# jbrea/BayesianOptimization.jl

Measured on AMD Instinct MI355X. Metric: acquisition-candidates/sec (N=3000,d=8), higher is better.
Workload: dtype f64

## Files before the change

### bayesianoptimization.jl_amd/csrc/bohip.hip

```cpp
#include "../../include/bohip.h"
#include "../../include/bohip_paths.h"
#include "../../include/bohip_fit.h"
#include "../../include/bohip_qei.h"
#include "../../include/bohip_acq.h"
#include "../../include/bohip_kg.h"
#include "../../include/bohip_ens.h"
#include "kernels_linalg.hip"
#include "kernels_chol.hip"
#include "kernels_exec.hip"
#include "kernels_score.hip"
#include "kernels_batch.hip"
#include "kernels_sample.hip"
#include "kernels_qei.hip"
#include "kernels_kg.hip"
#include "kernels_path.hip"
#include "kernels_ascent.hip"
#include "kernels_fit.hip"
#include "kernels_ens.hip"
#include "kernels_small.hip"
#include "direct_l.h"

#include <algorithm>
#include <atomic>
#include <chrono>
// ... 292 lines not shown
    HIPCHK(hipMalloc(&g->dr, (g->ld + 256) * 8));
    HIPCHK(hipMalloc(&g->dt, (g->ld + 256) * 8));
    HIPCHK(hipMalloc(&g->dApp, (size_t)APP_ROWS * g->ld * 8));
    {
        const size_t Tm = (size_t)(g->ld / TILE) + 1;
        HIPCHK(hipMalloc(&g->dchol_flags, chol_flag_words((int)std::min<size_t>(Tm, CHOL_DF_TCAP)) * sizeof(unsigned)));
        HIPCHK(hipMalloc(&g->dchol_idl, Tm * CH_PANELS * 256 * 8));
    }
    HIPCHK(hipMemsetAsync(g->dL, 0, mat, g->stream));
    HIPCHK(hipMemsetAsync(g->dW, 0, mat, g->stream));
    HIPCHK(hipMemsetAsync(g->dWT, 0, mat, g->stream));
    HIPCHK(hipMemsetAsync(g->dS, 0, mat, g->stream));
    if (g->n > 0) {
        HIPCHK(hipMemcpyAsync(g->dX, g->hX.data(), (size_t)g->n * g->d * 8, hipMemcpyHostToDevice, g->stream));
        HIPCHK(hipMemcpyAsync(g->dy, g->hy.data(), (size_t)g->n * 8, hipMemcpyHostToDevice, g->stream));
    }
    g->stale = true;
    return 0;
}

static int g_bulk_pieces = 4;
static int g_sample_mfma_min = 200;
static int g_path_mfma_min = 24;
static int g_split = 1;
static int g_asc_wg_nmax = 256;
static const double g_asc_first_step = 0.1;
static int g_asc_fold = 1;
static int g_asc_lockstep = 0;
static int g_small_m = 0;
static int g_small_r = -1;
static int g_inv_hi_h = 16;
static int g_chol_df = 1;
static bool g_chol_df_strict = false;
static bool g_chol_df_dump = false;
static int g_chol_df_tmax = 96;
static std::atomic<int> g_chol_df_skip{0}, g_chol_df_backoff{0};
static unsigned long long g_chol_spin_ticks = CH_SPIN_TICKS_DEFAULT;
static int g_chol_exec_patience_us = 1000;
static int g_chol_exec_fill_inv = 1;
static int g_chol_exec_inv_pairs = 0;
static std::atomic<int> g_chol_inv_grp_min{28};
static std::atomic<int> g_chol_inv_g{8};
static int g_chol_nsf = 3;
static int g_chol_exec_urgent = -1;
static int g_chol_exec_second = 1;
static int g_small_zero_copy = 1;
static int g_chol_exec_nbu = 2;
static int g_chol_exec_fast = -1;
static int g_chol_exec_pairs = -1;
static int g_chol_exec_wgs = -1;
static int g_append_alpha_inc = 1;
static int64_t g_chunk_rows_forced = 0;
static int g_prune_m = -1;
static int g_pa_order = 1;
static int launch_gemm_nt(bohip_gp* g, const GemmNTParams& p, int batch = 1, hipStream_t st = nullptr, bool hi = false) {
    if (p.mt <= 0 || p.nt64 <= 0 || p.kc <= 0 || batch <= 0) return 0;
    if (hi) hipLaunchKernelGGL(k_gemm_nt_hi, dim3(p.mt * p.nt64, batch), dim3(GEMM_THREADS_8), glds3_lds_bytes<4>(), st ? st : g->stream, p);
    else hipLaunchKernelGGL(k_gemm_nt, dim3(p.mt * p.nt64, batch), dim3(GEMM_THREADS_8), glds3_lds_bytes<4>(), st ? st : g->stream, p);
    HIPCHK(hipGetLastError());
    return 0;
}

static int device_cus();
static void read_dev_knobs() {
#if BOHIP_DEV_KNOBS
    struct Knob { const char* name; int* v; int lo, hi; };
    static int chunk_rows = 0, dump = 0;
    const Knob knobs[] = {
        {"BOHIP_CHOL_DF_TMAX", &g_chol_df_tmax, 0, CHOL_DF_TCAP}, {"BOHIP_INV_HI_H", &g_inv_hi_h, 0, 1 << 20},
        {"BOHIP_CHOL_EXEC_PAIRS", &g_chol_exec_pairs, -1, 64},
        {"BOHIP_CHOL_EXEC_URGENT", &g_chol_exec_urgent, 1, 1 << 20}, {"BOHIP_CHOL_NSF", &g_chol_nsf, 1, CH_NSF_MAX},
        {"BOHIP_CHOL_EXEC_PATIENCE_US", &g_chol_exec_patience_us, 0, 1 << 30}, {"BOHIP_CHOL_EXEC_FILL_INV", &g_chol_exec_fill_inv, 0, 1},
        {"BOHIP_CHOL_EXEC_INV_PAIRS", &g_chol_exec_inv_pairs, 0, 1}, {"BOHIP_CHOL_EXEC_WGS", &g_chol_exec_wgs, 1, 1 << 20},
        {"BOHIP_CHOL_EXEC_FAST", &g_chol_exec_fast, -1, 1 << 20},
        {"BOHIP_CHOL_EXEC_SECOND", &g_chol_exec_second, 0, 1}, {"BOHIP_SMALL_ZERO_COPY", &g_small_zero_copy, 0, 1}, {"BOHIP_CHOL_EXEC_NBU", &g_chol_exec_nbu, 0, 16}, {"BOHIP_CHUNK_ROWS", &chunk_rows, 0, 1 << 30},
        {"BOHIP_PRUNE_M", &g_prune_m, -1, 1 << 16}, {"BOHIP_PA_ORDER", &g_pa_order, 0, 1},
        {"BOHIP_APPEND_ALPHA_INC", &g_append_alpha_inc, 0, 1}, {"BOHIP_BULK_PIECES", &g_bulk_pieces, 0, 8}, {"BOHIP_SPLIT", &g_split, 0, 1},
        {"BOHIP_SMALL_R", &g_small_r, 0, SMALL_MAX}, {"BOHIP_SMALL_M", &g_small_m, 0, 1 << 20}, {"BOHIP_CHOL_DF_DUMP", &dump, 0, 1},
    };
    for (const Knob& k : knobs)
        if (const char* e = getenv(k.name)) *k.v = std::min(k.hi, std::max(k.lo, atoi(e)));
    g_chunk_rows_forced = chunk_rows;
    g_chol_df_dump = dump != 0;
#endif
}

static int one_time_kernel_setup() {
    static bool done_dev[64] = {false};
    int dev = 0;
    HIPCHK(hipGetDevice(&dev));
    bool& done = done_dev[dev & 63];
    if (done) return 0;
    HIPCHK(hipFuncSetAttribute((const void*)k_potf2_inv, hipFuncAttributeMaxDynamicSharedMemorySize, POTF2_LDS_BYTES));
    HIPCHK(hipFuncSetAttribute((const void*)k_gemm_nt, hipFuncAttributeMaxDynamicSharedMemorySize, glds3_lds_bytes<4>()));
    HIPCHK(hipFuncSetAttribute((const void*)k_trigemm_sq, hipFuncAttributeMaxDynamicSharedMemorySize, glds3_lds_bytes<4>()));
    HIPCHK(hipFuncSetAttribute((const void*)k_trigemm_sq_pa, hipFuncAttributeMaxDynamicSharedMemorySize, glds3_lds_bytes<4>()));
    HIPCHK(hipFuncSetAttribute((const void*)k_trigemm_rows, hipFuncAttributeMaxDynamicSharedMemorySize, RS_LDS_BYTES));
    HIPCHK(hipFuncSetAttribute((const void*)k_batch_cond<true>, hipFuncAttributeMaxDynamicSharedMemorySize, BATCH_LDS_MAX));
    HIPCHK(hipFuncSetAttribute((const void*)k_batch_cond<false>, hipFuncAttributeMaxDynamicSharedMemorySize, BATCH_LDS_MAX));
    HIPCHK(hipFuncSetAttribute((const void*)k_chol_chain, hipFuncAttributeMaxDynamicSharedMemorySize, CH_LDS_BYTES));
    HIPCHK(hipFuncSetAttribute((const void*)k_gemm_nt_hi, hipFuncAttributeMaxDynamicSharedMemorySize, glds3_lds_bytes<4>()));
    HIPCHK(hipFuncSetAttribute((const void*)k_chol_exec, hipFuncAttributeMaxDynamicSharedMemorySize, glds3_lds_bytes<4>()));
    HIPCHK(hipFuncSetAttribute((const void*)k_trimv_stream<TRIMV_D>, hipFuncAttributeMaxDynamicSharedMemorySize, trimv_lds_bytes(TRIMV_D)));
    HIPCHK(hipFuncSetAttribute((const void*)k_path_mfma<true>, hipFuncAttributeMaxDynamicSharedMemorySize, (int)path_mfma_lds_bytes(DMAX)));
    HIPCHK(hipFuncSetAttribute((const void*)k_path_mfma<false>, hipFuncAttributeMaxDynamicSharedMemorySize, (int)path_mfma_lds_bytes(DMAX)));
    HIPCHK(hipFuncSetAttribute((const void*)k_kg<true>, hipFuncAttributeMaxDynamicSharedMemorySize, (int)kg_lds_bytes(KG_RMAX)));
    HIPCHK(hipFuncSetAttribute((const void*)k_kg<false>, hipFuncAttributeMaxDynamicSharedMemorySize, (int)kg_lds_bytes(KG_RMAX)));
    if (const char* e = getenv("BOHIP_CHOL_DATAFLOW")) g_chol_df = atoi(e);
    if (const char* e = getenv("BOHIP_CHOL_SPIN_US")) g_chol_spin_ticks = 100ull * (unsigned long long)std::max(1, atoi(e));
    if (const char* e = getenv("BOHIP_CHOL_INV_G")) g_chol_inv_g = std::min(64, std::max(0, atoi(e)));
    if (const char* e = getenv("BOHIP_CHOL_INV_GRP_MIN")) g_chol_inv_grp_min = std::max(0, atoi(e));
    if (const char* e = getenv("BOHIP_ASC_WG_NMAX")) g_asc_wg_nmax = std::max(0, atoi(e));
    if (const char* e = getenv("BOHIP_ASC_LOCKSTEP")) { g_asc_lockstep = atoi(e) == 1; g_asc_fold = atoi(e) != 2; }
    if (const char* e = getenv("BOHIP_SAMPLE_MFMA_MIN")) g_sample_mfma_min = std::max(1, atoi(e));
    g_chol_df_strict = getenv("BOHIP_CHOL_DF_STRICT") != nullptr;
    read_dev_knobs();
    done = true;
    return 0;
}

static int launch_rows_trimv(bohip_gp* g, const double* W, int64_t N0, const double* rows, int P, double* out, int upper);
static int compute_alpha(bohip_gp* g) {
    const int64_t N = g->n;
    g->alpha_inc_run = 0;
    hipLaunchKernelGGL(k_sub_mean, dim3((N + 255) / 256), dim3(256), 0, g->stream, g->dy, g->beta, N, g->dr);
    HIPCHK(hipGetLastError());
    CHK(launch_rows_trimv(g, g->dW, N, g->dr, 1, g->dt, 0));
    CHK(launch_rows_trimv(g, g->dWT, N, g->dt, 1, g->dalpha, 1));
    HIPCHK(hipMemcpyAsync(g->dW + N * g->ld, g->dalpha, (size_t)N * 8, hipMemcpyDeviceToDevice, g->stream));
    return 0;
}

static int check_info(bohip_gp* g) {
    int info = 0;
    if (g->hpin) {
        int* pw = reinterpret_cast<int*>(g->hpin + 3 * SMALL_R) + 1;
        HIPCHK(hipMemcpyAsync(pw, g->dinfo, sizeof(int), hipMemcpyDeviceToHost, g->stream));
        HIPCHK(hipStreamSynchronize(g->stream));
        info = *pw;
    } else {
        HIPCHK(hipMemcpyAsync(&info, g->dinfo, sizeof(int), hipMemcpyDeviceToHost, g->stream));
        HIPCHK(hipStreamSynchronize(g->stream));
    }
    if (info != 0) {
        g->pivot = info;
        g->stale = true;
        return fail(BOHIP_E_NOTPD, "kernel matrix not positive definite at pivot " + std::to_string(info));
    }
    g->pivot = 0;
// ... 1142 lines not shown
static int prune_tiles(int T) {
    if (g_prune_m >= 0) return g_prune_m < T ? g_prune_m : 0;
    int m = 2;
    while ((double)m * (m + 1) < 0.02 * T * (T + 1)) ++m;
    return m < T ? m : 0;
}
static std::vector<int> rows_halves(const std::vector<int>& pieces) {
    std::vector<int> out;
    for (int c : pieces) {
        const int rt = c & 0xffff, mode = c >> 16;
        if (mode == PIECE_UPPER_SOLO) out.push_back(rt | 1 << 17);
        else { out.push_back(rt | 1 << 16); out.push_back(rt); }
    }
    std::stable_sort(out.begin(), out.end(), [](int a, int b) {
        return 8 * (a & 0xffff) + ((a >> 16) & 1) * 4 > 8 * (b & 0xffff) + ((b >> 16) & 1) * 4;
    });
    return out;
}
static int rows_halves_from(const std::vector<int>& hv, int t0) {
    int n = 0;
    while (n < (int)hv.size() && (hv[n] & 0xffff) >= t0) ++n;
    return n;
}
static int launch_trigemm_rows(bohip_gp* g, const double* KsT, const int* halves, int NH, const int* list, const unsigned* cnt,
                               int cnt_max, double* q, int64_t ldq, double* mu, int groups = 0, const PruneFinish* pf = nullptr,
                               unsigned* arrive = nullptr) {
    if (NH <= 0 || cnt_max <= 0) return 0;
    RowsParams rp{};
    rp.W = g->dW; rp.ldw = g->ld; rp.KsT = KsT; rp.ldk = g->ld; rp.list = list; rp.cnt = cnt; rp.cnt_max = cnt_max;
    rp.halves = halves; rp.NH = NH; rp.G = groups > 0 ? groups : (cnt_max + RS_COLS - 1) / RS_COLS;
    rp.alpha_row = g->n; rp.q = q; rp.ldq = ldq; rp.mu = mu;
    if (pf) { rp.finish = 1; rp.arrive = arrive; rp.pf = *pf; }
    hipLaunchKernelGGL(k_trigemm_rows, dim3((unsigned)(8 * ((NH + 7) / 8) * rp.G)), dim3(RS_THREADS), RS_LDS_BYTES, g->stream, rp);
    HIPCHK(hipGetLastError());
    return 0;
}
static int launch_trigemm_on(bohip_gp* g, const double* KsT, const int* pieces, int NP, int CT, double* q, int64_t ldq, double* mu_raw,
                             FuseParams fz) {
    const int n_local = (CT + 7) / 8;
    if (NP <= 0 || CT <= 0) return 0;
    if (g->timing && g->dclk) fz.clk = g->dclk;
    hipLaunchKernelGGL(k_trigemm_sq, dim3(8 * n_local * NP), dim3(GEMM_THREADS_8), glds3_lds_bytes<4>(), g->stream, g->dW, g->ld, KsT,
                       g->ld, pieces, NP, CT, g->n, q, ldq, mu_raw, (int64_t)0, nullptr, g->ld, fz);
    HIPCHK(hipGetLastError());
    return 0;
}
static std::vector<int> phase_a_jobs(const std::vector<int>& pieces, int m) {
    std::vector<int> out;
    for (int c : pieces)
        if ((c & 0xffff) < m) { out.push_back((c & 0xffff) | 1 << 16); out.push_back(c & 0xffff); }
    std::stable_sort(out.begin(), out.end(), [](int a, int b) {
        return 8 * (a & 0xffff) + (a >> 16) * 4 > 8 * (b & 0xffff) + (b >> 16) * 4;
    });
    if (g_pa_order == 1) std::rotate(out.begin(), out.begin() + out.size() / 3, out.begin() + 2 * (out.size() / 3));
    return out;
}
static int launch_phase_a(bohip_gp* g, const double* KsT, const int* jobs, int NJOBS, int CT, double* q, int64_t ldq) {
    const int n_local = (CT + 7) / 8;
    if (NJOBS <= 0 || CT <= 0) return 0;
    hipLaunchKernelGGL(k_trigemm_sq_pa, dim3(8 * n_local * NJOBS), dim3(GEMM_THREADS_8), glds3_lds_bytes<4>(), g->stream, g->dW, g->ld,
                       KsT, g->ld, jobs, CT, q, ldq, g->timing && g->dclk ? g->dclk : nullptr);
    HIPCHK(hipGetLastError());
    return 0;
}
static int pruned_pass(bohip_gp* g, const double* dXs, int64_t R, int m, const AcqParams& ap, Best* d_best, int64_t best_off,
                       double* ub_host = nullptr, bool long_form = false) {
    CHK(one_time_kernel_setup());
    if (!g->hprune_stat) {
        HIPCHK(hipHostMalloc((void**)&g->hprune_stat, 64, hipHostMallocDefault));
        g->hprune_stat[0] = 0u;
    }
    const int64_t N = g->n, Npad = round_up(N + 1, TILE), Rpad = round_up(R, TILE) + TILE, ld = g->ld;
    const int T = (int)(Npad / TILE);
    const int64_t P = Npad / 64;
    CHK(ensure_pieces(g, T, N));
    std::vector<int> pa, pb;
    for (int c : g->hpieces) ((c & 0xffff) < m ? pa : pb).push_back(c);
    if (m >= T) return fail(BOHIP_E_STATE, "pruned pass: the prefix holds the alpha row");
    for (int c : pa)
        if (c >> 16 != PIECE_WHOLE) return fail(BOHIP_E_STATE, "pruned pass: a half piece in the prefix");
    const std::vector<int> ph = phase_a_jobs(g->hpieces, m);
    auto al = [](size_t b) { return (b + 255) / 256 * 256; };
    const size_t o_ks = 0, o_q2 = o_ks + al((size_t)Rpad * ld * 8), o_mu2 = o_q2 + al((size_t)2 * T * Rpad * 8),
                 o_ub = o_mu2 + al((size_t)Rpad * 8), o_l1 = o_ub + al((size_t)Rpad * 8), o_l2 = o_l1 + al((size_t)PRUNE_K1 * 4),
                 o_mark = o_l2 + al((size_t)Rpad * 4), o_cnt = o_mark + al((size_t)Rpad * 4), o_rec = o_cnt + 256,
                 o_parts = o_rec + 256, o_pc = o_parts + al((size_t)2 * P * Rpad * 8), total = o_pc + al((5 * g->hpieces.size() + 8) * 4);
    bool fresh = false;
    if (g->pr_bytes < total) {
        fresh = true;
        if (g->dpr) { HIPCHK(hipStreamSynchronize(g->stream)); HIPCHK(hipFree(g->dpr)); g->dpr = nullptr; g->pr_bytes = 0; }
        HIPCHK(hipMalloc(&g->dpr, total));
        g->pr_bytes = total;
    }
    char* b = g->dpr;
    double *ks2 = (double*)(b + o_ks), *q2 = (double*)(b + o_q2), *mu2 = (double*)(b + o_mu2), *ub = (double*)(b + o_ub);
    int *l1 = (int*)(b + o_l1), *l2 = (int*)(b + o_l2), *mark = (int*)(b + o_mark), *pcs = (int*)(b + o_pc);
    const KstarParts kp{g->dW + N * ld, (double*)(b + o_parts), Rpad};
    unsigned* cnt = (unsigned*)(b + o_cnt);
    Best* rec = (Best*)(b + o_rec);
    const std::vector<int> hv = rows_halves(g->hpieces);
    const int nh = rows_halves_from(hv, m);
    std::vector<int> both = pa;
    both.insert(both.end(), pb.begin(), pb.end());
    both.insert(both.end(), hv.begin(), hv.end());
    both.insert(both.end(), ph.begin(), ph.end());
    if (fresh || g->hpr_pieces != both || g->pr_pieces_at != pcs) {
        g->pr_pieces_at = pcs;
        g->hpr_pieces = both;
        HIPCHK(hipMemcpyAsync(pcs, g->hpr_pieces.data(), both.size() * sizeof(int), hipMemcpyHostToDevice, g->stream));
    }
    if (g->timing && !g->dclk) {
        HIPCHK(hipMalloc(&g->dclk, 2 * sizeof(unsigned long long)));
        HIPCHK(hipMemsetAsync(g->dclk, 0, 2 * sizeof(unsigned long long), g->stream));
// ... 2340 lines not shown
```

### bayesianoptimization.jl_amd/csrc/gemm_core.h

```cpp
#pragma once
#ifndef BOHIP_TRACE
#define BOHIP_TRACE 0
#endif
#ifndef BOHIP_ABL
#define BOHIP_ABL 0
#endif
#include <type_traits>
#include "common.h"

namespace bohip {

typedef double d2 __attribute__((ext_vector_type(2)));

__device__ __forceinline__ double mfma444(double a, double b, double c) {
    return __builtin_amdgcn_mfma_f64_4x4x4f64(a, b, c, 0, 0, 0);
}

typedef __attribute__((address_space(3))) void* lds_void_ptr;
typedef const __attribute__((address_space(1))) void* gbl_void_ptr;
constexpr int GL_ROW = KC;

template <int NJ>
__device__ __forceinline__ void load_frags_swz(const double* ap, const double* bp, const int (&oa)[2], const int (&ob)[2],
                                               int S, d2 (&av)[8], d2 (&bv)[NJ]) {
// ... 36 lines not shown
template <int NJ>
__device__ __forceinline__ void mma_chunk_swz(const double* ap, const double* bp, const int (&oa)[2], const int (&ob)[2],
                                              double (&acc)[8][NJ]) {
    d2 a0[8], b0[NJ], a1[8], b1[NJ];
    load_frags_swz<NJ>(ap, bp, oa, ob, 0, a0, b0);
    __builtin_amdgcn_sched_barrier(0);
    load_frags_swz<NJ>(ap, bp, oa, ob, 1, a1, b1);
    __builtin_amdgcn_sched_barrier(0);
    mma_pair<NJ>(a0, b0, acc);
    __builtin_amdgcn_sched_barrier(0);
    mma_pair<NJ>(a1, b1, acc);
}

template <int NJ>
constexpr int glds3_lds_bytes() { return 3 * (TILE + 16 * NJ) * GL_ROW * 8; }

template <int NJ, int ABL, int XY>
__device__ __forceinline__ void chunk_mma(const double* ap, const double* bp, int skip, double (&acc)[8][NJ]) {
    d2 av[8], bv[NJ];
    const uint32_t pa = (uint32_t)(uintptr_t)(__attribute__((address_space(3))) const double*)ap;
    const uint32_t pb = (uint32_t)(uintptr_t)(__attribute__((address_space(3))) const double*)bp;
    if constexpr ((ABL & 2) != 0) {
#pragma unroll
        for (int j = 0; j < NJ; ++j) asm volatile("" : "=v"(bv[j]) : "v"(pb));
#pragma unroll
        for (int i = 0; i < 8; ++i) asm volatile("" : "=v"(av[i]) : "v"(pa));
    } else {
        bv[0] = ds_read128<0>(pb); bv[1] = ds_read128<1024>(pb); bv[2] = ds_read128<2048>(pb); bv[3] = ds_read128<3072>(pb);
        av[0] = ds_read128<0>(pa); av[1] = ds_read128<1024>(pa); av[2] = ds_read128<2048>(pa); av[3] = ds_read128<3072>(pa);
        av[4] = ds_read128<4096>(pa); av[5] = ds_read128<5120>(pa); av[6] = ds_read128<6144>(pa); av[7] = ds_read128<7168>(pa);
    }
    asm volatile("s_waitcnt lgkmcnt(7)" : "+v"(bv[0]), "+v"(bv[1]), "+v"(bv[2]), "+v"(bv[3]), "+v"(av[0]));
    if (skip <= 0) mma_row<NJ, XY>(av[0], bv, acc[0]);
    asm volatile("s_waitcnt lgkmcnt(6)" : "+v"(av[1]));
    if (skip <= 1) mma_row<NJ, XY>(av[1], bv, acc[1]);
    asm volatile("s_waitcnt lgkmcnt(5)" : "+v"(av[2]));
    if (skip <= 2) mma_row<NJ, XY>(av[2], bv, acc[2]);
    asm volatile("s_waitcnt lgkmcnt(4)" : "+v"(av[3]));
    if (skip <= 3) mma_row<NJ, XY>(av[3], bv, acc[3]);
    asm volatile("s_waitcnt lgkmcnt(3)" : "+v"(av[4]));
    if (skip <= 4) mma_row<NJ, XY>(av[4], bv, acc[4]);
    asm volatile("s_waitcnt lgkmcnt(2)" : "+v"(av[5]));
    if (skip <= 5) mma_row<NJ, XY>(av[5], bv, acc[5]);
    asm volatile("s_waitcnt lgkmcnt(1)" : "+v"(av[6]));
    if (skip <= 6) mma_row<NJ, XY>(av[6], bv, acc[6]);
    asm volatile("s_waitcnt lgkmcnt(0)" : "+v"(av[7]));
    if (skip <= 7) mma_row<NJ, XY>(av[7], bv, acc[7]);
}

constexpr int GEMM_THREADS_8 = 512;
#if BOHIP_TRACE
__device__ unsigned long long g_phase[8192 * 8 * 4];
#endif
template <int NJ, int ABL = 0, bool SWAVE = false, bool FOLD = true, bool ROWS64 = false>
__device__ __forceinline__ void gemm_tile_loop_glds3_ks(const double* __restrict__ A, int64_t lda,
                                                        const double* __restrict__ B, int64_t ldb, int kc_begin,
                                                        int kc_end, double* smem, double (&acc)[8][NJ],
                                                        int active_rows = TILE, int tri_kc = 1 << 30, int tid_in = -1,
                                                        int row_h = 0) {
    static_assert(NJ == 4, "piece distribution below assumes 16 + 8 DMA pieces per chunk");
    constexpr int AT = TILE * GL_ROW, BT = 16 * NJ * GL_ROW;
    const int tid = tid_in >= 0 ? tid_in : (int)threadIdx.x, lane = tid & 63, wave = SWAVE ? __builtin_amdgcn_readfirstlane(tid >> 6) : (tid >> 6);
    const int w4 = wave & 3;
    const int khalf = ROWS64 ? w4 >> 1 : wave >> 2, wr = ROWS64 ? wave >> 2 : w4 >> 1, wc = w4 & 1;
    double* As = smem;
    double* Bs = smem + 3 * AT;
    if (kc_begin >= kc_end) return;
    const int prow = lane >> 3, sseg = (lane & 7) ^ (lane >> 3);
    const double* a_src0 = A + (int64_t)(wave * 8 + prow) * lda + sseg * 2;
    const double* a_src1 = A + (int64_t)((wave + 8) * 8 + prow) * lda + sseg * 2;
    const double* b_src = B + (int64_t)(wave * 8 + prow) * ldb + sseg * 2;
    double* a_dst0 = As + wave * 8 * GL_ROW;
    double* a_dst1 = As + (wave + 8) * 8 * GL_ROW;
    double* b_dst = Bs + wave * 8 * GL_ROW;
    auto issue = [&](int kc, int buf) {
        __builtin_amdgcn_global_load_lds((gbl_void_ptr)(a_src0 + (int64_t)kc * KC), (lds_void_ptr)(a_dst0 + buf * AT), 16, 0, 0);
        __builtin_amdgcn_global_load_lds((gbl_void_ptr)(a_src1 + (int64_t)kc * KC), (lds_void_ptr)(a_dst1 + buf * AT), 16, 0, 0);
        __builtin_amdgcn_global_load_lds((gbl_void_ptr)(b_src + (int64_t)kc * KC), (lds_void_ptr)(b_dst + buf * BT), 16, 0, 0);
    };
    auto issue_h = [&](int kc, int buf) {
        __builtin_amdgcn_global_load_lds((gbl_void_ptr)(a_src0 + (int64_t)kc * KC), (lds_void_ptr)(a_dst0 + buf * AT), 16, 0, 0);
        __builtin_amdgcn_global_load_lds((gbl_void_ptr)(b_src + (int64_t)kc * KC), (lds_void_ptr)(b_dst + buf * BT), 16, 0, 0);
    };
    const int k = lane >> 4, b = (lane >> 2) & 3, t = lane & 3;
    const int r7a = 4 * (b >> 1) + t, r7b = 4 * (b & 1) + t;
    const int oa = ((4 * khalf + k) ^ r7a) << 1, ob = ((4 * khalf + k) ^ r7b) << 1;
    const bool half = !ROWS64 && active_rows <= TILE / 2;
    const int wre = half || ROWS64 ? 0 : wr;
    const int xy = __builtin_amdgcn_readfirstlane(half ? 1 + wr : 0);
    const int a_frag = (wre * 64 + r7a) * GL_ROW + oa, b_frag = (wc * 8 * NJ + r7b) * GL_ROW + ob;
    const bool wave_active = ROWS64 ? wr == 0 : half || wr * 64 < active_rows;
    const int skip0 = __builtin_amdgcn_readfirstlane(khalf - 8 * (ROWS64 ? row_h : wre));
    if (half || ROWS64) {
        issue_h(kc_begin, 0);
        if (kc_begin + 1 < kc_end) {
            issue_h(kc_begin + 1, 1);
            asm volatile("s_waitcnt vmcnt(2)" ::: "memory");
        } else {
            asm volatile("s_waitcnt vmcnt(0)" ::: "memory");
        }
    } else {
        issue(kc_begin, 0);
        if (kc_begin + 1 < kc_end) {
            issue(kc_begin + 1, 1);
            asm volatile("s_waitcnt vmcnt(3)" ::: "memory");
        } else {
            asm volatile("s_waitcnt vmcnt(0)" ::: "memory");
        }
    }
    __builtin_amdgcn_s_barrier();
    auto run = [&](auto xy_tag) {
        int cur = 0;
#if BOHIP_TRACE
        unsigned long long ph0 = 0, ph1 = 0, ph2 = 0, phn = 0;
#endif
        for (int kc = kc_begin; kc < kc_end; ++kc) {
#if BOHIP_TRACE
            const unsigned long long tA = __builtin_amdgcn_s_memtime();
#endif
            const int nxt2 = cur == 0 ? 2 : cur - 1;
            const bool more2 = kc + 2 < kc_end;
            constexpr bool HALF = decltype(xy_tag)::value != 0 || ROWS64;
            if (more2 && !(ABL & 1)) {
                if constexpr (HALF) issue_h(kc + 2, nxt2);
                else issue(kc + 2, nxt2);
            }
            if (wave_active) {
                const double* ap = As + cur * AT + a_frag;
                const double* bp = Bs + cur * BT + b_frag;
                const int skip = kc >= tri_kc ? 2 * (kc - tri_kc) + skip0 : 0;
                chunk_mma<NJ, ABL, decltype(xy_tag)::value>(ap, bp, skip, acc);
            }
            __builtin_amdgcn_sched_barrier(0);
#if BOHIP_TRACE
            const unsigned long long tB = __builtin_amdgcn_s_memtime();
            __builtin_amdgcn_sched_barrier(0);
#endif
            if (more2) {
                if constexpr (HALF) asm volatile("s_waitcnt vmcnt(2)" ::: "memory");
                else asm volatile("s_waitcnt vmcnt(3)" ::: "memory");
            } else {
                asm volatile("s_waitcnt vmcnt(0)" ::: "memory");
            }
            asm volatile("s_waitcnt lgkmcnt(0)" ::: "memory");
#if BOHIP_TRACE
            const unsigned long long tC = __builtin_amdgcn_s_memtime();
            __builtin_amdgcn_sched_barrier(0);
#endif
            if constexpr ((ABL & 4) == 0) __builtin_amdgcn_s_barrier();
            __builtin_amdgcn_sched_barrier(0);
#if BOHIP_TRACE
            const unsigned long long tD = __builtin_amdgcn_s_memtime();
            ph0 += tB - tA; ph1 += tC - tB; ph2 += tD - tC; phn += 1;
#endif
            cur = cur == 2 ? 0 : cur + 1;
        }
#if BOHIP_TRACE
        if (lane == 0 && blockIdx.x < 8192) {
            unsigned long long* o = g_phase + ((size_t)blockIdx.x * 8 + wave) * 4;
            o[0] = ph0; o[1] = ph1; o[2] = ph2; o[3] = phn;
        }
#endif
    };
    if constexpr (ROWS64) {
        run(std::integral_constant<int, 0>{});
    } else {
        if (xy == 0) run(std::integral_constant<int, 0>{});
        else if (xy == 1) run(std::integral_constant<int, 1>{});
        else run(std::integral_constant<int, 2>{});
    }
    if constexpr (!FOLD) return;
    double* xch = smem;
    const bool folds = !ROWS64 || wr == 0;
    if (khalf == 1 && folds) {
#pragma unroll
        for (int i = 0; i < 8; ++i)
#pragma unroll
            for (int j = 0; j < NJ; ++j) xch[(i * NJ + j) * 256 + (ROWS64 ? wc * 64 + lane : (tid & 255))] = acc[i][j];
    }
    __syncthreads();
    if (khalf == 0 && folds) {
#pragma unroll
        for (int i = 0; i < 8; ++i)
#pragma unroll
            for (int j = 0; j < NJ; ++j) acc[i][j] += xch[(i * NJ + j) * 256 + (ROWS64 ? wc * 64 + lane : tid)];
    }
    __syncthreads();
    if (half) {
        if (khalf == 0 && wr == 1) {
#pragma unroll
            for (int i = 0; i < 8; ++i)
#pragma unroll
                for (int j = 0; j < NJ; ++j) {
                    xch[(i * NJ + j) * 256 + (tid - 128)] = acc[i][j];
                    acc[i][j] = 0.0;
                }
        }
        __syncthreads();
        if (khalf == 0 && wr == 0) {
#pragma unroll
            for (int i = 0; i < 8; ++i)
#pragma unroll
                for (int j = 0; j < NJ; ++j) acc[i][j] += xch[(i * NJ + j) * 256 + tid];
        }
        __syncthreads();
    }
}

__device__ __forceinline__ int acc_row(int lane, int wr, int mi) {
    return wr * 64 + 8 * mi + 4 * (((lane >> 2) & 3) >> 1) + (lane >> 4);
}
template <int NJ>
__device__ __forceinline__ int acc_col(int lane, int wc, int nj) {
    return wc * 8 * NJ + 8 * nj + 4 * (((lane >> 2) & 3) & 1) + (lane & 3);
}

}
```

### bayesianoptimization.jl_amd/csrc/kernels_score.hip

```cpp
#include "gemm_core.h"
#include "acq_log.h"

namespace bohip {

template <bool LOW>
__device__ __forceinline__ double cov_from_r_fast(int fam, double sigma2, double r) {
    if constexpr (LOW) {
        return matern_lo_k(fam, sigma2, r);
    } else {
        if (fam == FAM_M52) {
            const double R = sqrt(r), s = sqrt(5.0) * R;
            return sigma2 * (1.0 + s + 5.0 / 3.0 * r) * exp(-s);
        }
        return sigma2 * exp(-0.5 * r);
    }
}

struct KstarParts {
    const double* alpha;
    double* parts;
    int64_t ldp;
};
__device__ __forceinline__ void swap32(double a, double b, double& x, double& y) {
    const unsigned long long ua = (unsigned long long)__double_as_longlong(a), ub = (unsigned long long)__double_as_longlong(b);
// ... 214 lines not shown
    }
}

__global__ __launch_bounds__(GEMM_THREADS_8, 4) void k_trigemm_sq(const double* __restrict__ W, int64_t ldw,
                                                                  const double* __restrict__ KsT, int64_t ldk,
                                                                  const int* __restrict__ pieces, int NP, int CT, int64_t alpha_row,
                                                                  double* __restrict__ q_part, int64_t ldq,
                                                                  double* __restrict__ mu_raw, int64_t r_off,
                                                                  double* __restrict__ VT, int64_t ldv, FuseParams fz) {
    extern __shared__ __attribute__((aligned(16))) double smem[];
#if BOHIP_TRACE
    const unsigned long long t_start = wall_clock64(), c_start = clock64();
    struct TraceEnd {
        unsigned long long t0, c0;
        __device__ ~TraceEnd() {
            if (threadIdx.x == 0) {
                unsigned hw, xcc;
                asm volatile("s_getreg_b32 %0, hwreg(HW_REG_HW_ID)" : "=s"(hw));
                asm volatile("s_getreg_b32 %0, hwreg(HW_REG_XCC_ID)" : "=s"(xcc));
                unsigned long long* t = g_trace + 6 * (size_t)blockIdx.x;
                t[0] = t0; t[1] = wall_clock64(); t[2] = hw; t[3] = xcc; t[4] = c0; t[5] = clock64();
            }
        }
    } trace_end{t_start, c_start};
#endif
    const int xcd = blockIdx.x & 7, slot = blockIdx.x >> 3;
    const int n_local = (CT + 7) >> 3;
    const int ct = xcd + 8 * (slot % n_local);
    if (ct >= CT) return;
    if (fz.live != nullptr && ct * CTILE >= (int)*fz.live) return;
    const int piece = __builtin_amdgcn_readfirstlane(pieces[slot / n_local]);
    __shared__ unsigned long long s_clk[2];
    if (fz.clk != nullptr && blockIdx.x % 33 == 0 && threadIdx.x == 0) { s_clk[0] = clock64(); s_clk[1] = wall_clock64(); }
    trigemm_job(piece & 0xffff, piece >> 16, ct, W, ldw, KsT, ldk, NP, alpha_row, q_part, ldq, mu_raw, r_off, VT, ldv, fz, smem,
                    (int)threadIdx.x);
    if (fz.clk != nullptr && blockIdx.x % 33 == 0 && threadIdx.x == 0) {
        atomicAdd(fz.clk, (unsigned long long)clock64() - s_clk[0]);
        atomicAdd(fz.clk + 1, (unsigned long long)wall_clock64() - s_clk[1]);
    }
}

__device__ __forceinline__ void trigemm_job_rows64(int rt, int hh, int ct, const double* __restrict__ W, int64_t ldw,
                                                   const double* __restrict__ KsT, int64_t ldk, double* __restrict__ q_part,
                                                   int64_t ldq, double* smem, int tid) {
    constexpr int NJ = 4, CW = CTILE;
    double acc[8][NJ];
#pragma unroll
    for (int i = 0; i < 8; ++i)
#pragma unroll
        for (int j = 0; j < NJ; ++j) acc[i][j] = 0.0;
    const int64_t row_base = (int64_t)rt * TILE + 64 * hh;
    const int tri_kc = rt * (TILE / KC);
    const int kc_end = tri_kc + (hh == 0 ? 4 : 8);
    gemm_tile_loop_glds3_ks<NJ, BOHIP_ABL, true, true, true>(W + row_base * ldw, ldw, KsT + (int64_t)ct * CW * ldk, ldk, 0, kc_end, smem,
                                                             acc, TILE / 2, tri_kc, tid, hh);
    const int lane = tid & 63, wave = tid >> 6, wc = wave & 1;
    __syncthreads();
    double* red = smem;
    if (wave < 2) {
#pragma unroll
        for (int nj = 0; nj < NJ; ++nj) {
            double s = 0.0;
#pragma unroll
            for (int mi = 0; mi < 8; ++mi) s = sq_step(s, acc[mi][nj]);
            s = sq_tree(s);
            if (lane < 8) red[wc * 8 * NJ + 8 * nj + lane] = s;
        }
    }
    __syncthreads();
    if (tid < CW)
        __hip_atomic_store(q_part + (int64_t)(2 * rt + hh) * ldq + (int64_t)ct * CW + tid, red[tid], __ATOMIC_RELAXED, __HIP_MEMORY_SCOPE_AGENT);
}

__global__ __launch_bounds__(GEMM_THREADS_8, 4) void k_trigemm_sq_pa(const double* __restrict__ W, int64_t ldw,
                                                                     const double* __restrict__ KsT, int64_t ldk,
                                                                     const int* __restrict__ jobs, int CT, double* __restrict__ q_part,
                                                                     int64_t ldq, unsigned long long* clk) {
    extern __shared__ __attribute__((aligned(16))) double smem[];
#if BOHIP_TRACE
    const unsigned long long t_start = wall_clock64(), c_start = clock64();
    struct TraceEnd {
        unsigned long long t0, c0;
        __device__ ~TraceEnd() {
            if (threadIdx.x == 0) {
                unsigned hw, xcc;
                asm volatile("s_getreg_b32 %0, hwreg(HW_REG_HW_ID)" : "=s"(hw));
                asm volatile("s_getreg_b32 %0, hwreg(HW_REG_XCC_ID)" : "=s"(xcc));
                unsigned long long* t = g_trace + 6 * (size_t)blockIdx.x;
                t[0] = t0; t[1] = wall_clock64(); t[2] = hw; t[3] = xcc; t[4] = c0; t[5] = clock64();
            }
        }
    } trace_end{t_start, c_start};
#endif
    const int xcd = blockIdx.x & 7, slot = blockIdx.x >> 3;
    const int n_local = (CT + 7) >> 3;
    const int ct = xcd + 8 * (slot % n_local);
    if (ct >= CT) return;
    const int job = __builtin_amdgcn_readfirstlane(jobs[slot / n_local]);
    __shared__ unsigned long long s_clk[2];
    if (clk != nullptr && blockIdx.x % 33 == 0 && threadIdx.x == 0) { s_clk[0] = clock64(); s_clk[1] = wall_clock64(); }
    trigemm_job_rows64(job & 0xffff, job >> 16, ct, W, ldw, KsT, ldk, q_part, ldq, smem, (int)threadIdx.x);
    if (clk != nullptr && blockIdx.x % 33 == 0 && threadIdx.x == 0) {
        atomicAdd(clk, (unsigned long long)clock64() - s_clk[0]);
        atomicAdd(clk + 1, (unsigned long long)wall_clock64() - s_clk[1]);
    }
}

__global__ __launch_bounds__(256) void k_split_combine_v(const double* __restrict__ PT, int64_t plane, int64_t ldp, int kz,
                                                         int64_t N, double* __restrict__ q, double* __restrict__ mu_raw,
                                                         double* __restrict__ VT, int64_t ldv) {
    __shared__ double red[256];
    const int r = blockIdx.x;
    const double* base = PT + (int64_t)r * ldp;
    double s = 0.0;
    for (int64_t i = threadIdx.x; i <= N; i += 256) {
        const int nsl = (int)(((i >> 7) + 1) * (TILE / KC) + kz - 1) / kz;
        double v = 0.0;
        for (int sl = 0; sl < nsl; ++sl) v += base[(int64_t)sl * plane + i];
        if (i < N) {
            s += v * v;
            if (VT) VT[(int64_t)r * ldv + i] = v;
        } else {
            mu_raw[r] = v;
        }
    }
    red[threadIdx.x] = s;
    __syncthreads();
// ... 887 lines not shown
```

Baseline: 29.69 million.

## Add deep-prefetch ring loop for 64-row phase-A triangular GEMM jobs

New measurement: 28.54 million. 3.9% lower.

```diff
diff --git a/bayesianoptimization.jl_amd/csrc/bohip.hip b/bayesianoptimization.jl_amd/csrc/bohip.hip
--- a/bayesianoptimization.jl_amd/csrc/bohip.hip
+++ b/bayesianoptimization.jl_amd/csrc/bohip.hip
@@ -368,7 +368,6 @@
 static int g_append_alpha_inc = 1;
 static int64_t g_chunk_rows_forced = 0;
 static int g_prune_m = -1;
-static int g_pa_order = 1;
 static int launch_gemm_nt(bohip_gp* g, const GemmNTParams& p, int batch = 1, hipStream_t st = nullptr, bool hi = false) {
     if (p.mt <= 0 || p.nt64 <= 0 || p.kc <= 0 || batch <= 0) return 0;
     if (hi) hipLaunchKernelGGL(k_gemm_nt_hi, dim3(p.mt * p.nt64, batch), dim3(GEMM_THREADS_8), glds3_lds_bytes<4>(), st ? st : g->stream, p);
@@ -390,7 +389,7 @@
         {"BOHIP_CHOL_EXEC_INV_PAIRS", &g_chol_exec_inv_pairs, 0, 1}, {"BOHIP_CHOL_EXEC_WGS", &g_chol_exec_wgs, 1, 1 << 20},
         {"BOHIP_CHOL_EXEC_FAST", &g_chol_exec_fast, -1, 1 << 20},
         {"BOHIP_CHOL_EXEC_SECOND", &g_chol_exec_second, 0, 1}, {"BOHIP_SMALL_ZERO_COPY", &g_small_zero_copy, 0, 1}, {"BOHIP_CHOL_EXEC_NBU", &g_chol_exec_nbu, 0, 16}, {"BOHIP_CHUNK_ROWS", &chunk_rows, 0, 1 << 30},
-        {"BOHIP_PRUNE_M", &g_prune_m, -1, 1 << 16}, {"BOHIP_PA_ORDER", &g_pa_order, 0, 1},
+        {"BOHIP_PRUNE_M", &g_prune_m, -1, 1 << 16},
         {"BOHIP_APPEND_ALPHA_INC", &g_append_alpha_inc, 0, 1}, {"BOHIP_BULK_PIECES", &g_bulk_pieces, 0, 8}, {"BOHIP_SPLIT", &g_split, 0, 1},
         {"BOHIP_SMALL_R", &g_small_r, 0, SMALL_MAX}, {"BOHIP_SMALL_M", &g_small_m, 0, 1 << 20}, {"BOHIP_CHOL_DF_DUMP", &dump, 0, 1},
     };
@@ -410,7 +409,7 @@
     HIPCHK(hipFuncSetAttribute((const void*)k_potf2_inv, hipFuncAttributeMaxDynamicSharedMemorySize, POTF2_LDS_BYTES));
     HIPCHK(hipFuncSetAttribute((const void*)k_gemm_nt, hipFuncAttributeMaxDynamicSharedMemorySize, glds3_lds_bytes<4>()));
     HIPCHK(hipFuncSetAttribute((const void*)k_trigemm_sq, hipFuncAttributeMaxDynamicSharedMemorySize, glds3_lds_bytes<4>()));
-    HIPCHK(hipFuncSetAttribute((const void*)k_trigemm_sq_pa, hipFuncAttributeMaxDynamicSharedMemorySize, glds3_lds_bytes<4>()));
+    HIPCHK(hipFuncSetAttribute((const void*)k_trigemm_sq_pa, hipFuncAttributeMaxDynamicSharedMemorySize, PA_LDS_BYTES));
     HIPCHK(hipFuncSetAttribute((const void*)k_trigemm_rows, hipFuncAttributeMaxDynamicSharedMemorySize, RS_LDS_BYTES));
     HIPCHK(hipFuncSetAttribute((const void*)k_batch_cond<true>, hipFuncAttributeMaxDynamicSharedMemorySize, BATCH_LDS_MAX));
     HIPCHK(hipFuncSetAttribute((const void*)k_batch_cond<false>, hipFuncAttributeMaxDynamicSharedMemorySize, BATCH_LDS_MAX));
@@ -1659,13 +1658,12 @@
     std::stable_sort(out.begin(), out.end(), [](int a, int b) {
         return 8 * (a & 0xffff) + (a >> 16) * 4 > 8 * (b & 0xffff) + (b >> 16) * 4;
     });
-    if (g_pa_order == 1) std::rotate(out.begin(), out.begin() + out.size() / 3, out.begin() + 2 * (out.size() / 3));
     return out;
 }
 static int launch_phase_a(bohip_gp* g, const double* KsT, const int* jobs, int NJOBS, int CT, double* q, int64_t ldq) {
     const int n_local = (CT + 7) / 8;
     if (NJOBS <= 0 || CT <= 0) return 0;
-    hipLaunchKernelGGL(k_trigemm_sq_pa, dim3(8 * n_local * NJOBS), dim3(GEMM_THREADS_8), glds3_lds_bytes<4>(), g->stream, g->dW, g->ld,
+    hipLaunchKernelGGL(k_trigemm_sq_pa, dim3(8 * n_local * NJOBS), dim3(GEMM_THREADS_8), PA_LDS_BYTES, g->stream, g->dW, g->ld,
                        KsT, g->ld, jobs, CT, q, ldq, g->timing && g->dclk ? g->dclk : nullptr);
     HIPCHK(hipGetLastError());
     return 0;
diff --git a/bayesianoptimization.jl_amd/csrc/gemm_core.h b/bayesianoptimization.jl_amd/csrc/gemm_core.h
--- a/bayesianoptimization.jl_amd/csrc/gemm_core.h
+++ b/bayesianoptimization.jl_amd/csrc/gemm_core.h
@@ -112,17 +112,16 @@
 #if BOHIP_TRACE
 __device__ unsigned long long g_phase[8192 * 8 * 4];
 #endif
-template <int NJ, int ABL = 0, bool SWAVE = false, bool FOLD = true, bool ROWS64 = false>
+template <int NJ, int ABL = 0, bool SWAVE = false, bool FOLD = true>
 __device__ __forceinline__ void gemm_tile_loop_glds3_ks(const double* __restrict__ A, int64_t lda,
                                                         const double* __restrict__ B, int64_t ldb, int kc_begin,
                                                         int kc_end, double* smem, double (&acc)[8][NJ],
-                                                        int active_rows = TILE, int tri_kc = 1 << 30, int tid_in = -1,
-                                                        int row_h = 0) {
+                                                        int active_rows = TILE, int tri_kc = 1 << 30, int tid_in = -1) {
     static_assert(NJ == 4, "piece distribution below assumes 16 + 8 DMA pieces per chunk");
     constexpr int AT = TILE * GL_ROW, BT = 16 * NJ * GL_ROW;
     const int tid = tid_in >= 0 ? tid_in : (int)threadIdx.x, lane = tid & 63, wave = SWAVE ? __builtin_amdgcn_readfirstlane(tid >> 6) : (tid >> 6);
     const int w4 = wave & 3;
-    const int khalf = ROWS64 ? w4 >> 1 : wave >> 2, wr = ROWS64 ? wave >> 2 : w4 >> 1, wc = w4 & 1;
+    const int khalf = wave >> 2, wr = w4 >> 1, wc = w4 & 1;
     double* As = smem;
     double* Bs = smem + 3 * AT;
     if (kc_begin >= kc_end) return;
@@ -145,13 +144,13 @@
     const int k = lane >> 4, b = (lane >> 2) & 3, t = lane & 3;
     const int r7a = 4 * (b >> 1) + t, r7b = 4 * (b & 1) + t;
     const int oa = ((4 * khalf + k) ^ r7a) << 1, ob = ((4 * khalf + k) ^ r7b) << 1;
-    const bool half = !ROWS64 && active_rows <= TILE / 2;
-    const int wre = half || ROWS64 ? 0 : wr;
+    const bool half = active_rows <= TILE / 2;
+    const int wre = half ? 0 : wr;
     const int xy = __builtin_amdgcn_readfirstlane(half ? 1 + wr : 0);
     const int a_frag = (wre * 64 + r7a) * GL_ROW + oa, b_frag = (wc * 8 * NJ + r7b) * GL_ROW + ob;
-    const bool wave_active = ROWS64 ? wr == 0 : half || wr * 64 < active_rows;
-    const int skip0 = __builtin_amdgcn_readfirstlane(khalf - 8 * (ROWS64 ? row_h : wre));
-    if (half || ROWS64) {
+    const bool wave_active = half || wr * 64 < active_rows;
+    const int skip0 = __builtin_amdgcn_readfirstlane(khalf - 8 * wre);
+    if (half) {
         issue_h(kc_begin, 0);
         if (kc_begin + 1 < kc_end) {
             issue_h(kc_begin + 1, 1);
@@ -180,7 +179,7 @@
 #endif
             const int nxt2 = cur == 0 ? 2 : cur - 1;
             const bool more2 = kc + 2 < kc_end;
-            constexpr bool HALF = decltype(xy_tag)::value != 0 || ROWS64;
+            constexpr bool HALF = decltype(xy_tag)::value != 0;
             if (more2 && !(ABL & 1)) {
                 if constexpr (HALF) issue_h(kc + 2, nxt2);
                 else issue(kc + 2, nxt2);
@@ -222,28 +221,23 @@
         }
 #endif
     };
-    if constexpr (ROWS64) {
-        run(std::integral_constant<int, 0>{});
-    } else {
-        if (xy == 0) run(std::integral_constant<int, 0>{});
-        else if (xy == 1) run(std::integral_constant<int, 1>{});
-        else run(std::integral_constant<int, 2>{});
-    }
+    if (xy == 0) run(std::integral_constant<int, 0>{});
+    else if (xy == 1) run(std::integral_constant<int, 1>{});
+    else run(std::integral_constant<int, 2>{});
     if constexpr (!FOLD) return;
     double* xch = smem;
-    const bool folds = !ROWS64 || wr == 0;
-    if (khalf == 1 && folds) {
+    if (khalf == 1) {
 #pragma unroll
         for (int i = 0; i < 8; ++i)
 #pragma unroll
-            for (int j = 0; j < NJ; ++j) xch[(i * NJ + j) * 256 + (ROWS64 ? wc * 64 + lane : (tid & 255))] = acc[i][j];
+            for (int j = 0; j < NJ; ++j) xch[(i * NJ + j) * 256 + (tid & 255)] = acc[i][j];
     }
     __syncthreads();
-    if (khalf == 0 && folds) {
+    if (khalf == 0) {
 #pragma unroll
         for (int i = 0; i < 8; ++i)
 #pragma unroll
-            for (int j = 0; j < NJ; ++j) acc[i][j] += xch[(i * NJ + j) * 256 + (ROWS64 ? wc * 64 + lane : tid)];
+            for (int j = 0; j < NJ; ++j) acc[i][j] += xch[(i * NJ + j) * 256 + tid];
     }
     __syncthreads();
     if (half) {
@@ -267,6 +261,162 @@
     }
 }
 
+constexpr int PA_DEPTH = 6;
+constexpr int PA_BUF = (64 + 64) * GL_ROW;
+constexpr int PA_LDS_BYTES = PA_DEPTH * PA_BUF * 8;
+template <int NJ>
+__device__ __forceinline__ void trigemm_loop_rows64_ahead(const double* __restrict__ A, int64_t lda, const double* __restrict__ B,
+                                                          int64_t ldb, int kc_end, double* smem, double (&acc)[8][NJ], int tri_kc,
+                                                          int tid, int row_h) {
+    static_assert(NJ == 4, "16 DMA pieces per chunk, one of A and one of B per wave");
+    static_assert(PA_DEPTH % 2 == 0 && PA_DEPTH >= 4, "a pair of chunks per barrier: the ring turns in pairs");
+    static_assert(PA_LDS_BYTES >= 8 * NJ * 256 * 8, "the khalf fold reuses the ring");
+    const int lane = tid & 63, wave = __builtin_amdgcn_readfirstlane(tid >> 6);
+    const int khalf = (wave >> 1) & 1, wc = wave & 1;
+    const int prow = lane >> 3, sseg = (lane & 7) ^ prow;
+    const double* a_src = A + (int64_t)(wave * 8 + prow) * lda + sseg * 2;
+    const double* b_src = B + (int64_t)(wave * 8 + prow) * ldb + sseg * 2;
+    double* a_dst = smem + wave * 8 * GL_ROW;
+    double* b_dst = smem + (64 + wave * 8) * GL_ROW;
+    auto issue = [&](int kc, int buf) {
+        kc = min(kc, kc_end - 1);
+        __builtin_amdgcn_global_load_lds((gbl_void_ptr)(a_src + (int64_t)kc * KC), (lds_void_ptr)(a_dst + buf * PA_BUF), 16, 0, 0);
+        __builtin_amdgcn_global_load_lds((gbl_void_ptr)(b_src + (int64_t)kc * KC), (lds_void_ptr)(b_dst + buf * PA_BUF), 16, 0, 0);
+    };
+    auto wait_left = [&](auto left) { asm volatile("s_waitcnt vmcnt(%0)" ::"n"(2 * decltype(left)::value) : "memory"); };
+    const int k = lane >> 4, b = (lane >> 2) & 3, t = lane & 3;
+    const int r7a = 4 * (b >> 1) + t, r7b = 4 * (b & 1) + t;
+    const int oa = ((4 * khalf + k) ^ r7a) << 1, ob = ((4 * khalf + k) ^ r7b) << 1;
+    const uint32_t ring0 = (uint32_t)(uintptr_t)(__attribute__((address_space(3))) const double*)smem;
+    const uint32_t fa = ring0 + (uint32_t)((r7a * GL_ROW + oa) * 8);
+    const uint32_t fb = ring0 + (uint32_t)(((64 + wc * 8 * NJ + r7b) * GL_ROW + ob) * 8);
+    const int skip0 = __builtin_amdgcn_readfirstlane(khalf - 8 * row_h);
+    auto frags = [&](int buf, d2 (&av)[8], d2 (&bv)[NJ]) {
+        const uint32_t pa = fa + (uint32_t)(buf * PA_BUF * 8), pb = fb + (uint32_t)(buf * PA_BUF * 8);
+        bv[0] = ds_read128<0>(pb); bv[1] = ds_read128<1024>(pb); bv[2] = ds_read128<2048>(pb); bv[3] = ds_read128<3072>(pb);
+        av[0] = ds_read128<0>(pa); av[1] = ds_read128<1024>(pa); av[2] = ds_read128<2048>(pa); av[3] = ds_read128<3072>(pa);
+        av[4] = ds_read128<4096>(pa); av[5] = ds_read128<5120>(pa); av[6] = ds_read128<6144>(pa); av[7] = ds_read128<7168>(pa);
+    };
+    auto landed = [&](d2 (&av)[8], d2 (&bv)[NJ]) {
+        asm volatile("s_waitcnt lgkmcnt(0)"
+                     : "+v"(bv[0]), "+v"(bv[1]), "+v"(bv[2]), "+v"(bv[3]), "+v"(av[0]), "+v"(av[1]), "+v"(av[2]), "+v"(av[3]), "+v"(av[4]),
+                       "+v"(av[5]), "+v"(av[6]), "+v"(av[7]));
+    };
+    auto mmas = [&](auto tri_tag, int kc, const d2 (&av)[8], const d2 (&bv)[NJ]) {
+        if constexpr (decltype(tri_tag)::value) {
+            const int skip = 2 * (kc - tri_kc) + skip0;
+#pragma unroll
+            for (int i = 0; i < 8; ++i)
+                if (skip <= i) mma_row<NJ, 0>(av[i], bv, acc[i]);
+        } else {
+#pragma unroll
+            for (int i = 0; i < 8; ++i) mma_row<NJ, 0>(av[i], bv, acc[i]);
+        }
+    };
+    auto mmas_reading = [&](int nbuf, const d2 (&av)[8], const d2 (&bv)[NJ], d2 (&nav)[8], d2 (&nbv)[NJ]) {
+        const uint32_t pa = fa + (uint32_t)(nbuf * PA_BUF * 8), pb = fb + (uint32_t)(nbuf * PA_BUF * 8);
+        mma_row<NJ, 0>(av[0], bv, acc[0]); nbv[0] = ds_read128<0>(pb); nbv[1] = ds_read128<1024>(pb); __builtin_amdgcn_sched_barrier(0);
+        mma_row<NJ, 0>(av[1], bv, acc[1]); nbv[2] = ds_read128<2048>(pb); nbv[3] = ds_read128<3072>(pb); __builtin_amdgcn_sched_barrier(0);
+        mma_row<NJ, 0>(av[2], bv, acc[2]); nav[0] = ds_read128<0>(pa); nav[1] = ds_read128<1024>(pa); __builtin_amdgcn_sched_barrier(0);
+        mma_row<NJ, 0>(av[3], bv, acc[3]); nav[2] = ds_read128<2048>(pa); nav[3] = ds_read128<3072>(pa); __builtin_amdgcn_sched_barrier(0);
+        mma_row<NJ, 0>(av[4], bv, acc[4]); nav[4] = ds_read128<4096>(pa); nav[5] = ds_read128<5120>(pa); __builtin_amdgcn_sched_barrier(0);
+        mma_row<NJ, 0>(av[5], bv, acc[5]); nav[6] = ds_read128<6144>(pa); nav[7] = ds_read128<7168>(pa); __builtin_amdgcn_sched_barrier(0);
+        mma_row<NJ, 0>(av[6], bv, acc[6]);
+        mma_row<NJ, 0>(av[7], bv, acc[7]);
+    };
+    auto run = [&](auto computes_tag) {
+        constexpr bool COMPUTES = decltype(computes_tag)::value;
+#pragma unroll
+        for (int p = 0; p < PA_DEPTH - 1; ++p) issue(p, p);
+        d2 av0[8], bv0[NJ], av1[8], bv1[NJ];
+        wait_left(std::integral_constant<int, PA_DEPTH - 2>{});
+        __builtin_amdgcn_s_barrier();
+        __builtin_amdgcn_sched_barrier(0);
+        if constexpr (COMPUTES) {
+            frags(0, av0, bv0);
+            landed(av0, bv0);
+            __builtin_amdgcn_sched_barrier(0);
+        }
+#if BOHIP_TRACE
+        unsigned long long ph0 = 0, ph1 = 0, ph2 = 0, phn = 0;
+#endif
+        int cur = 0;
+        auto pair = [&](auto tri_tag, int kc) {
+#if BOHIP_TRACE
+            const unsigned long long tA = __builtin_amdgcn_s_memtime();
+            __builtin_amdgcn_sched_barrier(0);
+#endif
+            wait_left(std::integral_constant<int, PA_DEPTH - 4>{});
+#if BOHIP_TRACE
+            const unsigned long long tB = __builtin_amdgcn_s_memtime();
+            __builtin_amdgcn_sched_barrier(0);
+#endif
+            __builtin_amdgcn_s_barrier();
+            __builtin_amdgcn_sched_barrier(0);
+#if BOHIP_TRACE
+            const unsigned long long tC = __builtin_amdgcn_s_memtime();
+            __builtin_amdgcn_sched_barrier(0);
+#endif
+            const int prev = cur == 0 ? PA_DEPTH - 1 : cur - 1, b1 = cur + 1, b2 = cur + 2 == PA_DEPTH ? 0 : cur + 2;
+            issue(kc + PA_DEPTH - 1, prev);
+            issue(kc + PA_DEPTH, cur);
+            if constexpr (COMPUTES && !decltype(tri_tag)::value) {
+                mmas_reading(b1, av0, bv0, av1, bv1);
+                landed(av1, bv1);
+                __builtin_amdgcn_sched_barrier(0);
+                mmas_reading(b2, av1, bv1, av0, bv0);
+                landed(av0, bv0);
+                __builtin_amdgcn_sched_barrier(0);
+            } else if constexpr (COMPUTES) {
+                frags(b1, av1, bv1);
+                __builtin_amdgcn_sched_barrier(0);
+                mmas(tri_tag, kc, av0, bv0);
+                landed(av1, bv1);
+                __builtin_amdgcn_sched_barrier(0);
+                frags(b2, av0, bv0);
+                __builtin_amdgcn_sched_barrier(0);
+                mmas(tri_tag, kc + 1, av1, bv1);
+                landed(av0, bv0);
+                __builtin_amdgcn_sched_barrier(0);
+            }
+#if BOHIP_TRACE
+            const unsigned long long tD = __builtin_amdgcn_s_memtime();
+            __builtin_amdgcn_sched_barrier(0);
+            ph0 += tD - tC; ph1 += tB - tA; ph2 += tC - tB; phn += 2;
+#endif
+            cur = b2;
+        };
+        int kc = 0;
+        for (; kc < tri_kc; kc += 2) pair(std::false_type{}, kc);
+        for (; kc < kc_end; kc += 2) pair(std::true_type{}, kc);
+        asm volatile("s_waitcnt vmcnt(0)" ::: "memory");
+#if BOHIP_TRACE
+        if (lane == 0 && blockIdx.x < 8192) {
+            unsigned long long* o = g_phase + ((size_t)blockIdx.x * 8 + wave) * 4;
+            o[0] = ph0; o[1] = ph1; o[2] = ph2; o[3] = phn;
+        }
+#endif
+    };
+    if (wave < 4) run(std::true_type{});
+    else run(std::false_type{});
+    __syncthreads();
+    double* xch = smem;
+    if (wave < 4 && khalf == 1) {
+#pragma unroll
+        for (int i = 0; i < 8; ++i)
+#pragma unroll
+            for (int j = 0; j < NJ; ++j) xch[(i * NJ + j) * 256 + wc * 64 + lane] = acc[i][j];
+    }
+    __syncthreads();
+    if (wave < 4 && khalf == 0) {
+#pragma unroll
+        for (int i = 0; i < 8; ++i)
+#pragma unroll
+            for (int j = 0; j < NJ; ++j) acc[i][j] += xch[(i * NJ + j) * 256 + wc * 64 + lane];
+    }
+    __syncthreads();
+}
+
 __device__ __forceinline__ int acc_row(int lane, int wr, int mi) {
     return wr * 64 + 8 * mi + 4 * (((lane >> 2) & 3) >> 1) + (lane >> 4);
 }
diff --git a/bayesianoptimization.jl_amd/csrc/kernels_score.hip b/bayesianoptimization.jl_amd/csrc/kernels_score.hip
--- a/bayesianoptimization.jl_amd/csrc/kernels_score.hip
+++ b/bayesianoptimization.jl_amd/csrc/kernels_score.hip
@@ -290,8 +290,7 @@
     const int64_t row_base = (int64_t)rt * TILE + 64 * hh;
     const int tri_kc = rt * (TILE / KC);
     const int kc_end = tri_kc + (hh == 0 ? 4 : 8);
-    gemm_tile_loop_glds3_ks<NJ, BOHIP_ABL, true, true, true>(W + row_base * ldw, ldw, KsT + (int64_t)ct * CW * ldk, ldk, 0, kc_end, smem,
-                                                             acc, TILE / 2, tri_kc, tid, hh);
+    trigemm_loop_rows64_ahead<NJ>(W + row_base * ldw, ldw, KsT + (int64_t)ct * CW * ldk, ldk, kc_end, smem, acc, tri_kc, tid, hh);
     const int lane = tid & 63, wave = tid >> 6, wc = wave & 1;
     __syncthreads();
     double* red = smem;
@@ -310,7 +309,7 @@
         __hip_atomic_store(q_part + (int64_t)(2 * rt + hh) * ldq + (int64_t)ct * CW + tid, red[tid], __ATOMIC_RELAXED, __HIP_MEMORY_SCOPE_AGENT);
 }
 
-__global__ __launch_bounds__(GEMM_THREADS_8, 4) void k_trigemm_sq_pa(const double* __restrict__ W, int64_t ldw,
+__global__ __launch_bounds__(GEMM_THREADS_8, 2) void k_trigemm_sq_pa(const double* __restrict__ W, int64_t ldw,
                                                                      const double* __restrict__ KsT, int64_t ldk,
                                                                      const int* __restrict__ jobs, int CT, double* __restrict__ q_part,
                                                                      int64_t ldq, unsigned long long* clk) {
```
